# mpitid/babble

Measured on AMD Instinct MI355X. Metric: consensus-ordered events/sec at N participants, higher is better.
Workload: dtype int32; 1 GPU; random-gossip DAG, 256 participants, 10000000 events per GPU, RunConsensus every K=256 events (39063 calls); participants=256, events_per_graph=10000000, k=256, graphs_per_gpu=1, parallelism=replicas1

## Files before the change

### babble_amd/csrc/hge_engine.hip

```cpp
#include <hip/hip_runtime.h>

#include <algorithm>
#include <chrono>
#include <cstdio>
#include <cstdlib>
#include <cstring>
#include <mutex>
#include <optional>
#include <string>
#include <thread>
#include <utility>
#include <vector>

#include "../../include/hge.h"
#include "hge_plan.h"
#include "hge_kernels.hip"
#include "hge_median_rows.hip"
#include "hge_wide32.hip"
#include "hge_coords.hip"
#include "hge_coords_win.hip"
#include "hge_rounds_coop.hip"
#include "hge_rounds_direct.hip"
#include "hge_walk_spec.hip"

// ... 375 lines not shown
    s_lwsum.free_();
    s_lwinit.free_();
    d_ts.free_();
    d_FDTD.free_();
    d_FDTW.free_();
    d_cts.free_();
    s_cts.free_();
    d_S.free_();
    d_ssb.free_();
    d_seeb.free_();
    s_H.free_();
    s_wdbg.free_();
    s_segfws.free_();
    d_coin.free_();
    d_wit.free_();
    d_fame.free_();
    s_dec.free_();
    s_decbit.free_();
    s_segdec.free_();
    s_keys.free_();
    s_keys2.free_();
    d_opcp.free_();
    d_tsch.free_();
    d_LA16.free_();
    d_ssc.free_();
    s_gran.free_();
    s_cH.free_();
    s_cS.free_();
    s_cT.free_();
    s_cM.free_();
    s_cn.free_();
    s_mb.free_();
    s_wpaths.free_();
    s_hist.free_();
    s_hstate.free_();
    s_hssc.free_();
    if (pin) (void)hipHostFree(pin);
    pin = nullptr;
    pin_cap = pin_used = 0;
    if (pin_ord) (void)hipHostFree(pin_ord);
    pin_ord = nullptr;
    pin_ord_dev = nullptr;
    pin_ord_cap = 0;
    cons_pin_n = 0;
    if (st) (void)hipStreamDestroy(st);
    st = nullptr;
  }

  void ensure_events(int64_t m) {
    if (m <= Ecap) return;
    int64_t cap = std::max<int64_t>(m, Ecap + Ecap / 2);
    d_creator.grow_keep(cap, n_dev, st);
    d_index.grow_keep(cap, n_dev, st);
    d_sp.grow_keep(cap, n_dev, st);
    d_op.grow_keep(cap, n_dev, st);
    d_ntx.grow_keep(cap, n_dev, st);
    d_ts.grow_keep(cap, n_dev, st);
    d_S.grow_keep(4 * cap, 4 * n_dev, st);
    d_coin.grow_keep(cap, n_dev, st);
    d_round.grow_keep(cap, n_coords, st);
    d_wit.grow_keep(cap, n_coords, st);
    d_rr.grow_keep(cap, n_coords, st, 0xFF);
    d_cts.grow_keep(cap, n_coords, st, 0);
    d_und.grow_keep(cap, n_und, st);
    Ecap = cap;
  }
// ... 938 lines not shown
      const char* mf = getenv("HGE_TEST_DIR_MEMBER_FLAG");
      int mflag_ep = mf ? atoi(mf) : 0;
      void* dargs[] = {&t, &olen, &len, &rstate, &rlo, &rlo_dev, &Rprev, &gran, &err, &ssc, &mb, &dbg,
                       &nostart, &nohist, &hmax, &nostart, &extra, &stall_ep, &force_exact, &mflag_ep, &paths,
                       &paths_next};
      prof_begin("k_rounds_direct");
      HIPCHK(launch_resident(direct_fn(), dim3(N), dim3(1024), dargs));
      prof_end();
    } else {
      void* args[] = {&t, &FDT, &olen, &len, &rstate, &rlo, &rlo_dev, &Rprev, &gran, &err, &ssc, &dbg};
      prof_begin("k_rounds_coop");
      HIPCHK(launch_resident((const void*)k_rounds_coop, dim3(N), dim3(COOP_BS), args));
      prof_end();
    }
    if (getenv("HGE_TEST_HANDOFF_FAIL")) {
      const int32_t one = 1, down = hge_plan::kRoundsStoodDown;
      h2d(err, &one, 4);
      h2d(rstate + 1, &down, 4);
    }
  }
  uint32_t* walk_mb() {
    s_mb.need((size_t)npow() * npow() + (size_t)npow() * npow() / 2);
    return s_mb.p;
  }
  DBuf<unsigned long long> s_wpaths;
  int walk_seq = 0;
  unsigned long long* walk_paths() {
    if (!s_wpaths.p) {
      s_wpaths.need(4);
      HIPCHK(hipMemset(s_wpaths.p, 0, 4 * sizeof(unsigned long long)));
    }
    walk_seq++;
    return s_wpaths.p + 2 * (walk_seq & 1);
  }
  static int walk_force_exact() {
    const char* e = getenv("HGE_TEST_DIR_EXACT");
    return e && atoi(e) != 0 ? 1 : 0;
  }
  const void* direct_fn() const {
    return N <= 64 ? (const void*)k_rounds_direct<1024, 64>
         : N <= 128 ? (const void*)k_rounds_direct<1024, 128>
                    : (const void*)k_rounds_direct<1024, 256>;
  }

  bool sweep16() const { return N > 32 && !wide32; }
  bool wla16() const { return N > 192 && (N & 3) == 0 && !wide32; }

  void to_wide32() {
    auto test_stop = [&](int stage) {
      if (test_w32_fail == stage) {
        test_w32_fail = 0;
        throw EngineError(HGE_ERR_DEVICE, "test: to_wide32 stopped after stage " + std::to_string(stage));
      }
    };
    ensure_fdtd();
    if (!(w32_done & 4)) {
      grow_chain_table(d_LA, ccap, false);
      w32_done |= 4;
      test_stop(1);
    }
    if (fdt16()) {
      const size_t n = (size_t)N * N * ccap;
      for (int which = 0; which < 2; which++) {
        if (w32_done & (1 << which)) continue;
        DBuf<int32_t>& b = which ? d_FD : d_FDT;
        int32_t* q = nullptr;
// ... 561 lines not shown
    oc.cand = b.cand;
    oc.ncand = ncand;
    oc.R_last = b.R_last;
    oc.recv = s_recv.p;
    oc.rr = s_rr.p;
    oc.cts = s_cts.p;
    oc.cnt = out_counts();
    oc.bpos = s_bpos.p;
    oc.total = out_word(hge_plan::ResultsLayout::kReceived);
    oc.blist = s_bpos.p + ncalls;
    oc.nblist = s_bpos.p + 2 * ncalls;
    oc.f_und = s_fund.p;
    oc.upos = s_upos.p;
    oc.nund = out_word(hge_plan::ResultsLayout::kUndetermined);
    oc.und_out = s_und2.p;
    oc.k1 = (OKey*)s_keys.p;
    oc.k2 = (OKey*)s_keys2.p;
    oc.ev_rr = d_rr.p;
    oc.ev_cts = d_cts.p;
    oc.ntx = out_tx(b);
    oc.ntxb = b.out.ntxb;
    oc.ids = out_ids(b);
    oc.pr = c_pr;
    oc.nrounds = b.do_fame ? b.w.nrounds() : 0;
    oc.clast = s_clast.p;
    oc.dec = s_dec.p;
    oc.nc = c_nc;
    oc.flags = c_flags;
    oc.lcr_old = lcr;
    oc.n_lo = (int)std::min<int64_t>(b.calls[0], n_coords);
    oc.n1 = (int)n_coords;
    oc.lcre_out = out_word(hge_plan::ResultsLayout::kLcrEvents);
    oc.front = front;
    return oc;
  }

  void ensure_wla(Batch& b) {
    if (b.wla_done || N <= 16 || b.R_last <= b.rr_lo) return;
    b.wla_done = true;
    d_WLA.need((size_t)Rcap * N * N);
    if (N > 64 && !wide32) d_WLR.need((size_t)Rcap * N * N);
    const Tables tw = tables();
    KLAUNCH(k_witness_la, dim3(div_up(N, 64), div_up(N, 64), b.R_last - b.rr_lo), dim3(256), 0, st, tw, b.rr_lo);
  }

  void order_stages(Batch& b) {
    const int ncalls = b.ncalls, ncand = b.ncand, nr = b.nr, nrounds = b.w.nrounds();
    s_out.need(b.out.total());
    const bool ocall = nr > 0 && ncalls == 1 && b.calls[0] >= n_coords && b.commit && N <= 16 && !b.spl &&
                       ncand <= SCAN_LDS && (int64_t)nr * group_lanes() <= 65536 && (nrounds == 0 || b.lcr_dev) &&
                       !getenv("HGE_NO_ORDER_CALL");
    if (!ocall) launch_pending_fame(b);
    if (nr == 0) {
      if (!b.hdr_done) out_init(b);
      s_recv.need(ncand);
      HIPCHK(hipMemsetAsync(s_recv.p, 0xFF, 4 * ncand, st));
      return;
    }
    SegInfo& si = b.si;
    si.pr_index = c_pidx;
    if (nrounds > 0) {
      si.pr_off = c_pr + nrounds;
      si.pr_cf = c_pr + 2 * nrounds;
      si.pr_len = c_pr + 3 * nrounds;
      si.clast = s_clast.p;
      si.dec = s_dec.p;
// ... 111 lines not shown
    if (!rlu)
      KLAUNCH(k_recv_flags, dim3(div_up(ncand, 256)), dim3(256), 0, st, s_recv.p, ncand,
              (int32_t*)nullptr, s_fund.p, b.commit ? 1 : 0, b.commit ? o_cc : (int32_t*)nullptr);
    if (!b.commit) {
      KLAUNCH(k_set_rr, dim3(div_up(ncand, 256)), dim3(256), 0, st, t, cand, ncand, s_recv.p,
              s_rr.p, s_cts.p, d_rr.p, d_cts.p, (unsigned long long*)out_word(hge_plan::ResultsLayout::kTx), 0);
      return;
    }
    s_bpos.need(2 * (size_t)ncalls + 2);
    int32_t* blist = s_bpos.p + ncalls;
    int32_t* nblist = s_bpos.p + 2 * ncalls;
    const bool lu = ncand <= 16384;
    s_und2.need(d_und.n);
    if (rlu)
      KLAUNCH(k_recv_list_und, dim3(2), dim3(1024), 0, st, (const int32_t*)s_recv.p, (int)ncand, o_cc, ncalls,
              s_bpos.p, o_cnt, blist, nblist, s_fund.p, s_upos.p, o_und, cand, s_und2.p);
    else if (lu)
      KLAUNCH(k_list_und, dim3(2), dim3(1024), 0, st, (const int32_t*)o_cc, ncalls, s_bpos.p, o_cnt, blist,
              nblist, (const int32_t*)s_fund.p, s_upos.p, (int)ncand, o_und, cand, s_und2.p);
    else
      KLAUNCH(k_bucket_list, dim3(1), dim3(1024), 0, st, (const int32_t*)o_cc, ncalls, s_bpos.p,
              o_cnt, blist, nblist);
    s_keys.need((size_t)ncand * sizeof(OKey));
    s_keys2.need((size_t)ncand * sizeof(OKey));
    OKey* k1 = (OKey*)s_keys.p;
    OKey* k2 = (OKey*)s_keys2.p;
    KLAUNCH(k_bucket_keys, dim3(div_up(ncand, 256)), dim3(256), 0, st, t, cand, ncand, s_recv.p,
            s_rr.p, s_cts.p, s_bpos.p, k1, d_rr.p, d_cts.p, out_tx(b));
    int32_t* ids_dst = out_ids(b);
    if (lazy_order && !b.order_out && !b.spl && pin_ord_dev) {
      ids_dst = pin_ord_dev;
      b.wrote_direct = true;
    }
    if (ncalls <= 8) {
      KLAUNCH(k_bucket_sort_all, dim3(ncalls), dim3(1024), 0, st, (const int32_t*)s_bpos.p,
              (const int32_t*)o_cc, (const int32_t*)blist, (const int32_t*)nblist, k1, k2, ids_dst);
    } else {
      KLAUNCH(k_bucket_sort, dim3(std::min(ncalls, 2048)), dim3(256), 0, st,
              (const int32_t*)s_bpos.p, (const int32_t*)o_cc, (const int32_t*)blist,
              (const int32_t*)nblist, k1, k2, ids_dst, 1);
      if (ncand > 512)
        KLAUNCH(k_bucket_sort_big, dim3(std::min(ncalls, n_cu())), dim3(1024), 0, st,
                (const int32_t*)s_bpos.p, (const int32_t*)o_cc, (const int32_t*)blist,
                (const int32_t*)nblist, (const OKey*)k1, k2, ids_dst);
    }
    if (!lu) {
      scan_large(s_fund.p, s_upos.p, ncand, o_und);
      KLAUNCH(k_scatter_und, dim3(div_up(ncand, 256)), dim3(256), 0, st, cand, ncand, s_fund.p, s_upos.p,
              s_und2.p);
    }
    std::swap(d_und, s_und2);
    b.got_order = true;
  }

  void persist_fame(Batch& b) {
    const int nrounds = b.w.nrounds();
    if (!b.do_fame || nrounds == 0 || b.order_ran != OrderRan::Stages) return;
    const Tables t = tables();
    int32_t* const lcre_out = out_word(hge_plan::ResultsLayout::kLcrEvents);
    if (b.lcr_dev) {
      const int64_t nfrom = std::min<int64_t>(b.calls[0], n_coords);
      const int nb_fp = (int)div_up((int64_t)nrounds * N, 256);
      KLAUNCH(k_fame_persist_lcre, dim3(nb_fp + std::max(1, div_up(n_coords - nfrom, 256))), dim3(256), 0, st, t,
              (const int32_t*)c_pr, (const int32_t*)(c_pr + nrounds), (const int32_t*)(c_pr + 2 * nrounds),
              (const int32_t*)(c_pr + 3 * nrounds), nrounds, (const int32_t*)s_clast.p, (const uint8_t*)s_dec.p,
              nb_fp, (const int64_t*)c_nc, (const int32_t*)c_flags, lcr, (int)nfrom, (int)n_coords, lcre_out);
      return;
    }
    fame_persist(t, nrounds);
    if (b.lcr_new > lcr) {
      b.lcr_up = true;
      const int r = b.lcr_new - 1;
      if (r >= 0) {
        const int64_t nfrom = std::min<int64_t>(b.calls[b.c_set], n_coords);
        KLAUNCH(k_lcre, dim3(std::max(1, div_up(n_coords - nfrom, 256))), dim3(256), 0, st, t,
                (int)nfrom, (int)n_coords, r, lcre_out);
      }
// ... 1311 lines not shown
  h->prof_names.clear();
  h->prof_ms.clear();
  h->prof_cnt.clear();
  return HGE_OK;
}

int hge_kernel_stats(hge_engine* h, int k, char* name, int namecap, double* total_ms,
                     int64_t* launches) {
  const int n = (int)h->prof_names.size();
  if (k < 0 || k >= n) return n;
  if (name && namecap > 0) {
    snprintf(name, namecap, "%s", h->prof_names[k].c_str());
  }
  if (total_ms) *total_ms = h->prof_ms[k];
  if (launches) *launches = h->prof_cnt[k];
  return n;
}

int32_t hge_coordinate_sweeps(hge_engine* h) { return h ? h->n_sweeps : -1; }

int hge_walk_select_paths(hge_engine* h, int64_t* narrow, int64_t* exact) {
  GUARD_BEGIN
  unsigned long long v[2] = {0, 0};
  if (h->s_wpaths.p && h->walk_seq > 0) {
    h->d2h(v, h->s_wpaths.p + 2 * (h->walk_seq & 1), 16);
    h->sync();
  }
  if (narrow) *narrow = (int64_t)v[0];
  if (exact) *exact = (int64_t)v[1];
  return HGE_OK;
  GUARD_END(h)
}

int64_t hge_host_syncs(hge_engine* h) { return h ? h->n_syncs : -1; }

int hge_stage_times(hge_engine* h, float* ms_out, int cap) {
  int n = std::min(cap, 7);
  for (int i = 0; i < n; i++) ms_out[i] = h->stage_ms[i];
  return n;
}

int64_t hge_frontier_fallbacks(hge_engine* h) {
  if (!h) return HGE_ERR_ARG;
  return h->n_frontier_fallbacks;
}

}
```

### babble_amd/csrc/hge_kernels.hip

```cpp
#include <hip/hip_runtime.h>
#include <stdint.h>

#define INF32 0x7FFFFFFF

namespace hge {

struct Tables {
  int N, NW, SM, ccap, Rcap;
  int NW2;
  uint32_t* LA16;
  const int32_t* creator;
  const int32_t* index;
  const int32_t* sp;
  const int32_t* op;
  const int64_t* ts;
  const uint64_t* S;
  const uint8_t* coin;
  const int32_t* ntx;
  int32_t* chain;
  int2* opcp;
  int64_t* tsch;
  int32_t* FDTD;
  uint8_t* FDTW;
  int32_t* WLA;
  uint16_t* WLA16;
  uint16_t* WLR;
  int32_t* LA;
  int32_t* FD;
  uint16_t* FD16;
  int32_t* round;
  uint8_t* wit;
  int32_t* C;
  int32_t* W;
  uint64_t* ssb;
// ... 2423 lines not shown
      sb[i] = k.b;
      ss[i] = (uint32_t)(k.s0 >> 32);
    } else {
      sr[i] = 0xFFFFFFFFu;
      sb[i] = ~0ull;
      ss[i] = 0xFFFFFFFFu;
    }
    ix[i] = (uint16_t)i;
  }
  __syncthreads();
  for (int size = 2; size <= P; size <<= 1) {
    for (int stride = size >> 1; stride > 0; stride >>= 1) {
      for (int i = tid; i < P / 2; i += T) {
        const int lo = 2 * stride * (i / stride) + (i % stride);
        const int hi = lo + stride;
        const bool up = ((lo & size) == 0);
        const int x = ix[lo], y = ix[hi];
        bool yl;
        if (sr[x] != sr[y]) yl = sr[y] < sr[x];
        else if (sb[x] != sb[y]) yl = sb[y] < sb[x];
        else if (ss[x] != ss[y]) yl = ss[y] < ss[x];
        else if (x >= n || y >= n) yl = y < x;
        else yl = okless(K[y], K[x]);
        if (yl == up) {
          ix[lo] = (uint16_t)y;
          ix[hi] = (uint16_t)x;
        }
      }
      bitonic_sync(stride, stride > 1 ? stride >> 1 : size);
    }
  }
}

__device__ void bucket_sort_big_one(int b, int nb, const int32_t* bend, const OKey* keys, OKey* tmp,
                                    int32_t* ids_out, uint64_t* sb, uint32_t* sr, uint32_t* ss, uint16_t* ix) {
  const int tid = threadIdx.x, T = blockDim.x;
  {
    const OKey* K = keys + (bend[b] - nb);
    int32_t* out = ids_out + (bend[b] - nb);
    if (nb <= BIG_SORT) {
      big_bitonic(K, nb, sb, sr, ss, ix);
      for (int i = tid; i < nb; i += T) out[i] = (int32_t)K[ix[i]].id;
      __syncthreads();
      return;
    }
    int32_t* S = (int32_t*)(tmp + (bend[b] - nb));
    const int na = (nb + 1) >> 1, nbb = nb - na;
    big_bitonic(K, na, sb, sr, ss, ix);
    for (int i = tid; i < na; i += T) S[i] = ix[i];
    __syncthreads();
    big_bitonic(K + na, nbb, sb, sr, ss, ix);
    for (int i = tid; i < nbb; i += T) S[na + i] = na + ix[i];
    __syncthreads();
    const int32_t* A = S;
    const int32_t* B = S + na;
    const int k0 = (int)((int64_t)nb * tid / T), k1 = (int)((int64_t)nb * (tid + 1) / T);
    int lo = max(0, k0 - nbb), hi = min(k0, na);
    while (lo < hi) {
      const int i = (lo + hi) >> 1;
      if (okless(K[A[i]], K[B[k0 - i - 1]])) lo = i + 1;
      else hi = i;
    }
    int i = lo, j = k0 - lo;
    for (int k = k0; k < k1; k++) {
      const bool takeA = j >= nbb || (i < na && okless(K[A[i]], K[B[j]]));
      out[k] = (int32_t)K[takeA ? A[i++] : B[j++]].id;
    }
    __syncthreads();
  }
}

__global__ void __launch_bounds__(1024) k_bucket_sort_big(const int32_t* bend, const int32_t* bcnt,
                                                          const int32_t* list, const int32_t* nlist,
                                                          const OKey* keys, OKey* tmp, int32_t* ids_out) {
  __shared__ uint64_t sb[BIG_SORT];
  __shared__ uint32_t sr[BIG_SORT], ss[BIG_SORT];
  __shared__ uint16_t ix[BIG_SORT];
  for (int li = blockIdx.x; li < *nlist; li += gridDim.x) {
    const int b = list[li];
    const int nb = bcnt[b];
    if (nb <= 512 || nb > 2 * BIG_SORT) continue;
    bucket_sort_big_one(b, nb, bend, keys, tmp, ids_out, sb, sr, ss, ix);
  }
}

__global__ void __launch_bounds__(1024) k_bucket_sort_all(const int32_t* bend, const int32_t* bcnt,
                                                          const int32_t* list, const int32_t* nlist,
                                                          OKey* keys, OKey* tmp, int32_t* ids_out) {
  constexpr size_t BIG_LDS = (size_t)BIG_SORT * (8 + 4 + 4 + 2);
  constexpr size_t POOL = BIG_LDS > sizeof(SortChunk<SORT_CH>) ? BIG_LDS : sizeof(SortChunk<SORT_CH>);
  __shared__ __attribute__((aligned(16))) unsigned char pool[POOL];
  uint64_t* sb = (uint64_t*)pool;
  uint32_t* sr = (uint32_t*)(pool + (size_t)BIG_SORT * 8);
  uint32_t* ss = (uint32_t*)(pool + (size_t)BIG_SORT * 12);
  uint16_t* ix = (uint16_t*)(pool + (size_t)BIG_SORT * 16);
  SortChunk<SORT_CH>& sc = *(SortChunk<SORT_CH>*)pool;
  for (int li = blockIdx.x; li < *nlist; li += gridDim.x) {
    const int b = list[li];
    const int nb = bcnt[b];
    if (nb > 512 && nb <= 2 * BIG_SORT) bucket_sort_big_one(b, nb, bend, keys, tmp, ids_out, sb, sr, ss, ix);
    else bucket_sort_one(b, bend, bcnt, keys, tmp, ids_out, false, sc);
    __syncthreads();
  }
}

__global__ void k_scatter_und(const int32_t* cand, int ncand, const int32_t* f_und,
                              const int32_t* pos, int32_t* und) {
  const int q = blockIdx.x * blockDim.x + threadIdx.x;
  if (q >= ncand || !f_und[q]) return;
  und[pos[q]] = cand[q];
}

__global__ void k_set_rr(Tables t, const int32_t* cand, int ncand, const int32_t* recv_call,
                         const int32_t* rr, const int64_t* cts, int32_t* ev_rr, int64_t* ev_cts,
                         unsigned long long* ntx_sum, int commit) {
  const int q = blockIdx.x * blockDim.x + threadIdx.x;
  const bool rec = q < ncand && recv_call[q] >= 0;
  unsigned long long tx = 0;
  if (rec) {
    const int x = cand[q];
    ev_rr[x] = rr[q];
    ev_cts[x] = cts[q];
    tx = (unsigned long long)t.ntx[x];
  }
  if (!commit) return;
  for (int o = 32; o > 0; o >>= 1) tx += __shfl_xor(tx, o);
  if ((threadIdx.x & 63) == 0 && tx) atomicAdd(ntx_sum, tx);
}

__global__ void k_split_filter(const int32_t* cand, int ncand, int32_t* recv_call, int c_lo, int c_hi,
                               int32_t guard, int32_t* flag) {
  const int q = blockIdx.x * blockDim.x + threadIdx.x;
  bool bad = false;
// ... 95 lines not shown
  if ((int)blockIdx.x < nb_fp) fame_persist_body(t, pr_round, pr_off, pr_cf, pr_len, nrounds, clast, dec, blockIdx.x);
  else lcre_dev_body(t, nc, flags, lcr_old, n_lo, n1, out, blockIdx.x - nb_fp);
}

struct OrderCall {
  SegInfo si;
  int rr_lo, nr;
  const int32_t* segoff;
  int32_t *segcnt, *seg_call, *seg_round;
  uint8_t* seg_dec;
  uint64_t* seg_fws;
  int32_t* theta;
  const int32_t* cand;
  int ncand, R_last;
  int32_t *recv, *rr;
  int64_t* cts;
  int32_t *cnt, *bpos, *total, *blist, *nblist;
  int32_t *f_und, *upos, *nund, *und_out;
  OKey *k1, *k2;
  int32_t* ev_rr;
  int64_t* ev_cts;
  unsigned long long* ntx;
  int ntxb;
  int32_t* ids;
  const int32_t* pr;
  int nrounds;
  const int32_t* clast;
  const uint8_t* dec;
  const int64_t* nc;
  const int32_t* flags;
  int lcr_old, n_lo, n1;
  int32_t* lcre_out;
  int front;
};
constexpr size_t OC_BIG_LDS = (size_t)BIG_SORT * (8 + 4 + 4 + 2);
constexpr size_t OC_POOL = OC_BIG_LDS > sizeof(SortChunk<SORT_CH>) ? OC_BIG_LDS : sizeof(SortChunk<SORT_CH>);
static_assert(OC_POOL >= sizeof(int) * (SCAN_LDS + SCAN_LDS / 16), "the scan borrows the sort pool");
template <int G>
__device__ __forceinline__ void order_call_body(const Tables& t, const OrderCall& o, unsigned char* pool) {
  __shared__ int s_cnt;
  __shared__ unsigned long long s_tx[16];
  const int tid = threadIdx.x, T = blockDim.x;
  if (o.front) {
    for (int64_t b = 0; b < (int64_t)o.nr * G; b += T)
      segments_group<G, 1>(t, b + tid, o.rr_lo, o.nr, 1, nullptr, o.si, o.segoff, o.segcnt, o.seg_call,
                           o.seg_round, o.seg_dec, o.seg_fws, o.theta);
    __syncthreads();
    for (int q = tid; q < o.ncand; q += T)
      round_received_item<1>(t, q, o.cand, o.ncand, nullptr, 1, 0, o.rr_lo, o.R_last, o.segoff, o.segcnt,
                             o.seg_call, o.seg_dec, o.seg_fws, o.theta, o.recv, o.rr, o.cts, nullptr);
  }
  if (tid == 0) s_cnt = 0;
  __syncthreads();
  int c = 0;
  for (int q = tid; q < o.ncand; q += T) c += o.recv[q] >= 0 ? 1 : 0;
  for (int s2 = 32; s2 > 0; s2 >>= 1) c += __shfl_xor(c, s2);
  if ((tid & 63) == 0 && c) atomicAdd(&s_cnt, c);
  for (int q = tid; q < o.ncand; q += T) o.f_und[q] = o.recv[q] == -1 ? 1 : 0;
  __syncthreads();
  if (tid == 0) o.cnt[0] = s_cnt;
  __syncthreads();
  bucket_list_body(o.cnt, 1, o.bpos, o.total, o.blist, o.nblist);
  __syncthreads();
  scan_small_core(o.f_und, o.upos, o.ncand, o.nund, o.cand, o.und_out, (int*)pool);
  __syncthreads();
  unsigned long long tx = 0;
  for (int b = 0; b < o.ncand; b += T)
    tx += bucket_key_item(t, b + tid, o.cand, o.ncand, o.recv, o.rr, o.cts, o.bpos, o.k1, o.ev_rr, o.ev_cts);
  if ((tid & 63) == 0) s_tx[tid >> 6] = tx;
  __syncthreads();
  if (tid == 0) {
    unsigned long long bt = 0;
    for (int w = 0; w < T / 64; w++) bt += s_tx[w];
    o.ntx[0] = bt;
  }
  for (int i = 1 + tid; i < o.ntxb; i += T) o.ntx[i] = 0;
  __syncthreads();
  {
    uint64_t* sb = (uint64_t*)pool;
    uint32_t* sr = (uint32_t*)(pool + (size_t)BIG_SORT * 8);
    uint32_t* ss = (uint32_t*)(pool + (size_t)BIG_SORT * 12);
    uint16_t* ix = (uint16_t*)(pool + (size_t)BIG_SORT * 16);
    SortChunk<SORT_CH>& sc = *(SortChunk<SORT_CH>*)pool;
    const int nl = *o.nblist;
    for (int li = 0; li < nl; li++) {
      const int b = o.blist[li];
      const int nb = o.cnt[b];
      if (nb > 512 && nb <= 2 * BIG_SORT) bucket_sort_big_one(b, nb, o.bpos, o.k1, o.k2, o.ids, sb, sr, ss, ix);
      else bucket_sort_one(b, o.bpos, o.cnt, o.k1, o.k2, o.ids, false, sc);
      __syncthreads();
    }
  }
  if (o.nrounds > 0) {
    const int np = o.nrounds;
    for (int b = 0; (int64_t)b * T < (int64_t)np * t.N; b++)
      fame_persist_body(t, o.pr, o.pr + np, o.pr + 2 * np, o.pr + 3 * np, np, o.clast, o.dec, b);
    for (int b = 0; b == 0 || b * T < o.n1 - o.n_lo; b++)
      lcre_dev_body(t, o.nc, o.flags, o.lcr_old, o.n_lo, o.n1, o.lcre_out, b);
  }
}
template <int G>
__global__ void __launch_bounds__(1024) k_order_call(Tables t, OrderCall o) {
  __shared__ __attribute__((aligned(16))) unsigned char pool[OC_POOL];
  order_call_body<G>(t, o, pool);
}
template <int G>
__global__ void __launch_bounds__(1024) k_consensus_call(Tables t, FameCall f, OrderCall o) {
  __shared__ __attribute__((aligned(16))) unsigned char pool[OC_POOL];
  fame_call_body<G, 1, true>(t, f);
  __syncthreads();
  order_call_body<G>(t, o, pool);
}

struct DynCall {
  int lcr, ncand, Rcap;
  int64_t n_c;
  const int32_t* rstate;
  const int32_t* minw;
  int64_t* c_nc;
  int32_t *c_Rc, *c_Lc, *c_flags, *c_pr, *c_pidx, *c_sgo;
  uint8_t *dec, *decbit;
// ... 143 lines not shown
```

### babble_amd/engine.py

```python
import ctypes
import os

import numpy as np

_ROOT = os.path.dirname(os.path.dirname(os.path.abspath(__file__)))
LIB_PATH = os.environ.get("HGE_LIB", os.path.join(_ROOT, "build", "libhge.so"))

HGE_NONE = -1
HGE_UNKNOWN = -2

ERRORS = {
    -1: "Could not find fake creator id",
    -2: "Self-parent not known",
    -3: "Self-parent has different creator",
    -4: "Other-parent not known",
    -5: "Self-parent not last known event by creator",
    -6: "Event index does not match the creator's chain position",
    -7: "Chain capacity exceeded",
    -11: "too late",
    -12: "not found",
}
HGE_ERR_CAPACITY = -7
HGE_ERR_TOO_LATE = -11
HGE_ERR_NOT_FOUND = -12
# ... 6 lines not shown

class HgeEvent(ctypes.Structure):
    _fields_ = [
        ("creator", ctypes.c_int32),
        ("index", ctypes.c_int32),
        ("self_parent", ctypes.c_int32),
        ("other_parent", ctypes.c_int32),
        ("timestamp_ns", ctypes.c_int64),
        ("s", ctypes.c_uint8 * 32),
        ("hash", ctypes.c_uint8 * 32),
        ("n_tx", ctypes.c_int32),
        ("reserved", ctypes.c_int32),
    ]


EVENT_DTYPE = np.dtype([
    ("creator", "<i4"), ("index", "<i4"), ("self_parent", "<i4"), ("other_parent", "<i4"),
    ("timestamp_ns", "<i8"), ("s", "u1", (32,)), ("hash", "u1", (32,)), ("n_tx", "<i4"),
    ("reserved", "<i4"),
])
assert EVENT_DTYPE.itemsize == ctypes.sizeof(HgeEvent)

EXPORTS = [
    "hge_create", "hge_destroy", "hge_last_error", "hge_reset", "hge_insert_events",
    "hge_divide_rounds", "hge_decide_fame", "hge_decide_round_received", "hge_find_order",
    "hge_run_consensus", "hge_replay", "hge_replay_prepare", "hge_replay_run",
    "hge_replay_fetch", "hge_replay_order", "hge_event_count", "hge_participants", "hge_rounds",
    "hge_last_consensus_round", "hge_last_committed_round_events",
    "hge_consensus_transactions", "hge_consensus_count", "hge_consensus_events",
    "hge_undetermined", "hge_known", "hge_round_of", "hge_is_witness", "hge_round_witness",
    "hge_fame", "hge_round_events", "hge_round_received", "hge_consensus_timestamp",
    "hge_consensus_timestamp_sources",
    "hge_ancestor", "hge_self_ancestor", "hge_see", "hge_strongly_see",
    "hge_oldest_self_ancestor_to_see", "hge_coordinates", "hge_coordinate_sweeps", "hge_walk_select_paths", "hge_host_syncs", "hge_frontier_fallbacks",
    "hge_stage_times",
    "hge_set_profiling", "hge_reset_kernel_stats", "hge_kernel_stats",
    "hge_consensus_log", "hge_event_rounds", "hge_event_received", "hge_set_cache_size",
    "hge_cache_size", "hge_participant_events", "hge_participant_event", "hge_last_from",
    "hge_diff", "hge_wire_info", "hge_read_wire_parents", "hge_parent_round", "hge_round_inc",
    "hge_round_diff", "hge_set_round", "hge_round_event_ids", "hge_split_begin", "hge_frontier_guess",
    "hge_frontier_walk", "hge_split_finish", "hge_frontier_rows", "hge_split_plan", "hge_split_exchange", "hge_split_run", "hge_split_emulate",
    "hge_verify_events", "hge_sha256_batch", "hge_ingest", "hge_fame_table",
    "hge_sha256_batch_device", "hge_ecdsa_p256_verify_digests_device", "hge_verify_events_device",
    "hge_ingest_device", "hge_device",
    "hge_store_create", "hge_store_destroy", "hge_store_set_event", "hge_store_has_event",
    "hge_store_participant_events", "hge_store_participant_event", "hge_store_last_from",
    "hge_store_known", "hge_store_add_consensus_event", "hge_store_consensus_events",
    "hge_store_consensus_count", "hge_store_set_round", "hge_store_get_round", "hge_store_rounds",
    "hge_store_round_witnesses", "hge_store_round_events",
    "hge_batch_create", "hge_batch_destroy", "hge_batch_last_error", "hge_batch_add", "hge_batch_stage",
    "hge_batch_run", "hge_batch_graphs", "hge_batch_info", "hge_batch_results", "hge_batch_kernel_ms",
    "hge_batch_fallbacks", "hge_batch_set_delivery", "hge_batch_delivery", "hge_batch_commits_view",
    "hge_gob_encode_wire_events", "hge_gob_decode_wire_events", "hge_gob_encode_event_body",
]

_lib = None


class BatchCommits(ctypes.Structure):
    _fields_ = [("ids", ctypes.POINTER(ctypes.c_int32)), ("rr", ctypes.POINTER(ctypes.c_int32)),
                ("cts", ctypes.POINTER(ctypes.c_int64)), ("counts", ctypes.POINTER(ctypes.c_int64)),
                ("ordered", ctypes.c_int64), ("calls", ctypes.c_int64)]


class _HostView:

    def __init__(self, owner, pointer, n, typestr):
# ... 36 lines not shown
        getattr(L, f).argtypes = [vp, P(i32), i64, P(i64)]
    L.hge_replay.argtypes = [vp, ctypes.c_void_p, i64, P(i64), i64, P(i32), P(i32), i64, P(i64),
                             P(i64)]
    L.hge_replay_prepare.argtypes = [vp, ctypes.c_void_p, i64, P(i64), i64, P(i32)]
    L.hge_replay_run.argtypes = [vp, P(i64)]
    L.hge_replay_fetch.argtypes = [vp, P(i32), i64, P(i64)]
    L.hge_replay_order.argtypes = [vp, P(P(i32)), P(i64)]
    for f in ("hge_event_count", "hge_consensus_transactions", "hge_consensus_count"):
        getattr(L, f).argtypes = [vp]
        getattr(L, f).restype = i64
    for f in ("hge_participants", "hge_rounds", "hge_last_consensus_round",
              "hge_last_committed_round_events"):
        getattr(L, f).argtypes = [vp]
        getattr(L, f).restype = i32
    for f in ("hge_consensus_events", "hge_undetermined"):
        getattr(L, f).argtypes = [vp, P(i32), i64]
        getattr(L, f).restype = i64
    L.hge_known.argtypes = [vp, P(i32)]
    for f in ("hge_round_of", "hge_is_witness", "hge_round_events", "hge_round_received"):
        getattr(L, f).argtypes = [vp, i32]
        getattr(L, f).restype = i32
    L.hge_consensus_timestamp.argtypes = [vp, i32]
    L.hge_consensus_timestamp.restype = i64
    for f in ("hge_round_witness", "hge_fame", "hge_ancestor", "hge_self_ancestor", "hge_see",
              "hge_strongly_see", "hge_oldest_self_ancestor_to_see"):
        getattr(L, f).argtypes = [vp, i32, i32]
        getattr(L, f).restype = i32
    L.hge_coordinates.argtypes = [vp, i32, P(i32), P(i32)]
    L.hge_stage_times.argtypes = [vp, P(ctypes.c_float), ctypes.c_int]
    L.hge_coordinate_sweeps.restype = ctypes.c_int32
    L.hge_coordinate_sweeps.argtypes = [vp]
    if hasattr(L, "hge_walk_select_paths"):
        L.hge_walk_select_paths.argtypes = [vp, P(i64), P(i64)]
    if hasattr(L, "hge_gob_encode_wire_events"):
        L.hge_gob_encode_wire_events.argtypes = [vp, i64, P(ctypes.c_uint8), P(i64), i32, P(ctypes.c_uint8), i64,
                                                 P(i64)]
        L.hge_gob_decode_wire_events.argtypes = [P(ctypes.c_uint8), i64, vp, i64, P(ctypes.c_uint8), i64, P(i64),
                                                 i64, P(i64), P(i64), P(i64)]
        L.hge_gob_encode_event_body.argtypes = [vp, P(ctypes.c_uint8), P(i64), P(ctypes.c_uint8), P(i64), i32,
                                                P(ctypes.c_uint8), i64, P(i64)]
    if hasattr(L, "hge_host_syncs"):
        L.hge_host_syncs.restype = i64
        L.hge_host_syncs.argtypes = [vp]
    L.hge_frontier_fallbacks.restype = i64
    L.hge_frontier_fallbacks.argtypes = [vp]
    L.hge_consensus_log.argtypes = [vp, i64, P(i32), i64]
    L.hge_consensus_log.restype = i64
    L.hge_event_rounds.argtypes = [vp, P(i32), P(ctypes.c_uint8), i64]
    L.hge_event_received.argtypes = [vp, P(i32), P(i64), i64]
    L.hge_consensus_timestamp_sources.argtypes = [vp, P(i32), i64, P(i32)]
    L.hge_fame_table.argtypes = [vp, i32, P(ctypes.c_int8)]
    L.hge_fame_table.restype = i32
    L.hge_set_cache_size.argtypes = [vp, i64]
    L.hge_cache_size.argtypes = [vp]
    L.hge_cache_size.restype = i64
    L.hge_participant_events.argtypes = [vp, i32, i64, P(i32), i64, P(i64)]
    L.hge_participant_event.argtypes = [vp, i32, i64]
    L.hge_participant_event.restype = i32
    L.hge_last_from.argtypes = [vp, i32]
    L.hge_last_from.restype = i32
    L.hge_diff.argtypes = [vp, P(i32), P(i32), i64, P(i64)]
    L.hge_wire_info.argtypes = [vp, i32, P(i32)]
    L.hge_read_wire_parents.argtypes = [vp, i32, i32, i32, i32, P(i32), P(i32)]
    L.hge_parent_round.argtypes = [vp, i32]
    L.hge_parent_round.restype = i32
    L.hge_round_inc.argtypes = [vp, i32]
# ... 475 lines not shown
    def split_finish(self, rows, ssc, natural):
        rows = np.ascontiguousarray(rows, np.int32)
        ssc = np.ascontiguousarray(ssc, np.uint64)
        n = ctypes.c_int64()
        self._check(self.L.hge_split_finish(self.h, _p32(rows),
                                            ssc.ctypes.data_as(ctypes.POINTER(ctypes.c_uint64)),
                                            len(rows), 1 if natural else 0, ctypes.byref(n)))
        self._nordered = n.value
        return n.value

    def set_profiling(self, on=True):
        self.L.hge_set_profiling(self.h, 1 if on else 0)
        self.L.hge_reset_kernel_stats(self.h)

    def kernel_stats(self):
        out = {}
        n = self.L.hge_kernel_stats(self.h, -1, None, 0, None, None)
        buf = ctypes.create_string_buffer(128)
        for k in range(n):
            ms = ctypes.c_double()
            cnt = ctypes.c_int64()
            self.L.hge_kernel_stats(self.h, k, buf, 128, ctypes.byref(ms), ctypes.byref(cnt))
            out[buf.value.decode()] = (ms.value, cnt.value)
        return out

    def coordinate_sweeps(self):
        return self.L.hge_coordinate_sweeps(self.h)

    def walk_select_paths(self):
        nar, ex = ctypes.c_int64(), ctypes.c_int64()
        self._check(self.L.hge_walk_select_paths(self.h, ctypes.byref(nar), ctypes.byref(ex)))
        return nar.value, ex.value

    def host_syncs(self):
        return int(self.L.hge_host_syncs(self.h))

    def frontier_fallbacks(self):
        return int(self.L.hge_frontier_fallbacks(self.h))

    def stage_times(self):
        out = (ctypes.c_float * 7)()
        n = self.L.hge_stage_times(self.h, out, 7)
        return list(out)[:n]

    def event_count(self):
        return self.L.hge_event_count(self.h)

    def rounds(self):
        return self.L.hge_rounds(self.h)

    def last_consensus_round(self):
        r = self.L.hge_last_consensus_round(self.h)
        return None if r < 0 else r

    def last_committed_round_events(self):
        return self.L.hge_last_committed_round_events(self.h)

    def consensus_transactions(self):
        return self.L.hge_consensus_transactions(self.h)

    def consensus_events(self):
        m = self.L.hge_consensus_events(self.h, None, 0)
        out = np.zeros(max(1, m), np.int32)
        self.L.hge_consensus_events(self.h, _p32(out), m)
        return out[:m]

# ... 271 lines not shown
```

### include/hge.h

```cpp
#ifndef HGE_H
#define HGE_H

#include <stdint.h>

#ifdef __cplusplus
extern "C" {
#endif

typedef struct hge_engine hge_engine;

enum hge_status {
  HGE_OK = 0,
  HGE_ERR_CREATOR = -1,
  HGE_ERR_SELF_PARENT_UNKNOWN = -2,
  HGE_ERR_SELF_PARENT_CREATOR = -3,
  HGE_ERR_OTHER_PARENT_UNKNOWN = -4,
  HGE_ERR_SELF_PARENT_NOT_LAST = -5,
  HGE_ERR_INDEX = -6,
  HGE_ERR_CAPACITY = -7,
  HGE_ERR_ARG = -8,
  HGE_ERR_DEVICE = -9,
  HGE_ERR_INTERNAL = -10,
  HGE_ERR_TOO_LATE = -11,
  HGE_ERR_NOT_FOUND = -12,
// ... 175 lines not shown
typedef struct {
  int64_t unix_sec;
  int32_t nsec;
  int16_t offset_min;
  int16_t set;
} hge_gob_time;
typedef struct {
  int64_t self_parent_index, other_parent_creator_id, other_parent_index, creator_id, index;
  hge_gob_time timestamp;
  uint8_t r[32], s[32];
  int32_t r_set, s_set;
  int64_t tx_first;
  int32_t tx_count, pad;
} hge_wire_event;
typedef struct {
  int32_t tx_count, n_parents;
  const uint8_t* creator;
  int64_t creator_len;
  hge_gob_time timestamp;
  int64_t index;
} hge_gob_body;
int hge_gob_encode_wire_events(const hge_wire_event* ev, int64_t n, const uint8_t* tx, const int64_t* tx_off,
                               int32_t first_type_id, uint8_t* out, int64_t cap, int64_t* n_out);
int hge_gob_decode_wire_events(const uint8_t* buf, int64_t len, hge_wire_event* ev, int64_t cap_ev, uint8_t* tx,
                               int64_t cap_bytes, int64_t* tx_off, int64_t cap_tx, int64_t* n_ev, int64_t* n_tx,
                               int64_t* n_bytes);
int hge_gob_encode_event_body(const hge_gob_body* body, const uint8_t* tx, const int64_t* tx_off,
                              const uint8_t* parents, const int64_t* parent_off, int32_t first_type_id,
                              uint8_t* out, int64_t cap, int64_t* n_out);

int hge_stage_times(hge_engine* h, float* ms_out, int cap);
int32_t hge_coordinate_sweeps(hge_engine* h);
int hge_walk_select_paths(hge_engine* h, int64_t* narrow, int64_t* exact);
int64_t hge_host_syncs(hge_engine* h);
int64_t hge_frontier_fallbacks(hge_engine* h);
int hge_set_profiling(hge_engine* h, int on);
int hge_reset_kernel_stats(hge_engine* h);
int hge_kernel_stats(hge_engine* h, int k, char* name, int namecap, double* total_ms,
                     int64_t* launches);

#ifdef __cplusplus
}
#endif
#endif
```

Baseline: 225.7 million events/s.

## Sort big buckets with packed 64-bit keys and register bitonic network

Adds a packed-key bitonic sort for large buckets. The round, b and upper s0 fields are range-compressed into one 64-bit word plus a 16-bit index, and the sort runs mostly in registers with DPP and permlane exchanges, using LDS only for transposes. Ties fall back to full OKey comparison, and buckets whose ranges don't fit fall back to the old index bitonic. k_bucket_sort_big now claims buckets dynamically through an atomic counter, and path counters are exposed via hge_sort_paths. The cost is extra reduction passes, tie-break global reads, and atomics per bucket.

```diff
diff --git a/babble_amd/csrc/hge_engine.hip b/babble_amd/csrc/hge_engine.hip
--- a/babble_amd/csrc/hge_engine.hip
+++ b/babble_amd/csrc/hge_engine.hip
@@ -431,6 +431,7 @@
     s_cn.free_();
     s_mb.free_();
     s_wpaths.free_();
+    s_spaths.free_();
     s_hist.free_();
     s_hstate.free_();
     s_hssc.free_();
@@ -1435,6 +1436,20 @@
     }
     walk_seq++;
     return s_wpaths.p + 2 * (walk_seq & 1);
+  }
+  DBuf<unsigned long long> s_spaths;
+  int sort_seq = 0;
+  bool sort_counted = false;
+  SortCtl sort_ctl() {
+    if (!s_spaths.p) {
+      s_spaths.need(8);
+      HIPCHK(hipMemset(s_spaths.p, 0, 8 * sizeof(unsigned long long)));
+    }
+    sort_seq++;
+    sort_counted = true;
+    const char* e = getenv("HGE_TEST_SORT_INDEX");
+    return SortCtl{s_spaths.p + 4 * (sort_seq & 1), s_spaths.p + 4 * ((sort_seq + 1) & 1),
+                   e && atoi(e) != 0 ? 1 : 0};
   }
   static int walk_force_exact() {
     const char* e = getenv("HGE_TEST_DIR_EXACT");
@@ -2062,6 +2077,7 @@
     oc.n1 = (int)n_coords;
     oc.lcre_out = out_word(hge_plan::ResultsLayout::kLcrEvents);
     oc.front = front;
+    oc.sort = sort_ctl();
     return oc;
   }
 
@@ -2239,9 +2255,10 @@
       ids_dst = pin_ord_dev;
       b.wrote_direct = true;
     }
+    sort_counted = false;
     if (ncalls <= 8) {
       KLAUNCH(k_bucket_sort_all, dim3(ncalls), dim3(1024), 0, st, (const int32_t*)s_bpos.p,
-              (const int32_t*)o_cc, (const int32_t*)blist, (const int32_t*)nblist, k1, k2, ids_dst);
+              (const int32_t*)o_cc, (const int32_t*)blist, (const int32_t*)nblist, k1, k2, ids_dst, sort_ctl());
     } else {
       KLAUNCH(k_bucket_sort, dim3(std::min(ncalls, 2048)), dim3(256), 0, st,
               (const int32_t*)s_bpos.p, (const int32_t*)o_cc, (const int32_t*)blist,
@@ -2249,7 +2266,7 @@
       if (ncand > 512)
         KLAUNCH(k_bucket_sort_big, dim3(std::min(ncalls, n_cu())), dim3(1024), 0, st,
                 (const int32_t*)s_bpos.p, (const int32_t*)o_cc, (const int32_t*)blist,
-                (const int32_t*)nblist, (const OKey*)k1, k2, ids_dst);
+                (const int32_t*)nblist, (const OKey*)k1, k2, ids_dst, sort_ctl());
     }
     if (!lu) {
       scan_large(s_fund.p, s_upos.p, ncand, o_und);
@@ -3627,6 +3644,19 @@
   GUARD_END(h)
 }
 
+int hge_sort_paths(hge_engine* h, int64_t* packed, int64_t* index) {
+  GUARD_BEGIN
+  unsigned long long v[2] = {0, 0};
+  if (h->s_spaths.p && h->sort_counted) {
+    h->d2h(v, h->s_spaths.p + 4 * (h->sort_seq & 1), 16);
+    h->sync();
+  }
+  if (packed) *packed = (int64_t)v[0];
+  if (index) *index = (int64_t)v[1];
+  return HGE_OK;
+  GUARD_END(h)
+}
+
 int64_t hge_host_syncs(hge_engine* h) { return h ? h->n_syncs : -1; }
 
 int hge_stage_times(hge_engine* h, float* ms_out, int cap) {
diff --git a/babble_amd/csrc/hge_kernels.hip b/babble_amd/csrc/hge_kernels.hip
--- a/babble_amd/csrc/hge_kernels.hip
+++ b/babble_amd/csrc/hge_kernels.hip
@@ -1,5 +1,7 @@
 #include <hip/hip_runtime.h>
 #include <stdint.h>
+
+#include "hge_sortkey.h"
 
 #define INF32 0x7FFFFFFF
 
@@ -2489,26 +2491,252 @@
   }
 }
 
-__device__ void bucket_sort_big_one(int b, int nb, const int32_t* bend, const OKey* keys, OKey* tmp,
-                                    int32_t* ids_out, uint64_t* sb, uint32_t* sr, uint32_t* ss, uint16_t* ix) {
-  const int tid = threadIdx.x, T = blockDim.x;
+constexpr size_t BIG_LDS = (size_t)BIG_SORT * (8 + 4 + 4 + 2);
+
+__device__ __forceinline__ bool pk_less(uint64_t wa, uint32_t ia, uint64_t wb, uint32_t ib, const OKey* K, int n) {
+  if (wa != wb) return wa < wb;
+  if (ia >= (uint32_t)n || ib >= (uint32_t)n) return ia < ib;
+  const uint64_t* x = (const uint64_t*)&K[ia];
+  const uint64_t* y = (const uint64_t*)&K[ib];
+#pragma unroll 1
+  for (int f = 0; f < 6; f++) {
+    const uint64_t xf = x[f], yf = y[f];
+    if (xf != yf) return xf < yf;
+  }
+  return K[ia].id < K[ib].id;
+}
+static_assert(sizeof(OKey) == 56 && offsetof(OKey, id) == 48, "pk_less walks a .. s3 as six words");
+
+template <int CTRL>
+__device__ __forceinline__ uint32_t pk_dpp(uint32_t v) {
+  return (uint32_t)__builtin_amdgcn_mov_dpp((int)v, CTRL, 0xF, 0xF, true);
+}
+template <int X>
+__device__ __forceinline__ uint32_t pk_xor(uint32_t v, int lane) {
+  if constexpr (X == 1) {
+    return pk_dpp<0xB1>(v);
+  } else if constexpr (X == 2) {
+    return pk_dpp<0x4E>(v);
+  } else if constexpr (X == 4) {
+    return pk_dpp<0x1B>(pk_dpp<0x141>(v));
+  } else if constexpr (X == 8) {
+    return pk_dpp<0x128>(v);
+  } else if constexpr (X == 16) {
+    const auto r = __builtin_amdgcn_permlane16_swap(v, v, false, false);
+    return (lane & 16) ? r[0] : r[1];
+  } else {
+    const auto r = __builtin_amdgcn_permlane32_swap(v, v, false, false);
+    return (lane & 32) ? r[0] : r[1];
+  }
+}
+
+template <int E, int X>
+__device__ __forceinline__ void pk_lane_stage_x(uint64_t (&w)[E], uint32_t (&id)[E], int lane, uint32_t pos, int size,
+                                                const OKey* K, int n) {
+  const bool want_min = ((lane & X) == 0) == ((pos & (uint32_t)size) == 0);
+#pragma unroll
+  for (int e = 0; e < E; e++) {
+    const uint64_t ow = (uint64_t)pk_xor<X>((uint32_t)w[e], lane) | ((uint64_t)pk_xor<X>((uint32_t)(w[e] >> 32), lane) << 32);
+    const uint32_t oi = pk_xor<X>(id[e], lane);
+    const bool take = pk_less(ow, oi, w[e], id[e], K, n) == want_min;
+    w[e] = take ? ow : w[e];
+    id[e] = take ? oi : id[e];
+  }
+}
+template <int E>
+__device__ __forceinline__ void pk_lane_stage(uint64_t (&w)[E], uint32_t (&id)[E], int x, int lane, uint32_t pos,
+                                              int size, const OKey* K, int n) {
+  switch (x) {
+    case 1: pk_lane_stage_x<E, 1>(w, id, lane, pos, size, K, n); break;
+    case 2: pk_lane_stage_x<E, 2>(w, id, lane, pos, size, K, n); break;
+    case 4: pk_lane_stage_x<E, 4>(w, id, lane, pos, size, K, n); break;
+    case 8: pk_lane_stage_x<E, 8>(w, id, lane, pos, size, K, n); break;
+    case 16: pk_lane_stage_x<E, 16>(w, id, lane, pos, size, K, n); break;
+    default: pk_lane_stage_x<E, 32>(w, id, lane, pos, size, K, n); break;
+  }
+}
+
+template <int E>
+__device__ __forceinline__ bool packed_bitonic(const OKey* K, int n, int P, unsigned char* pool, uint16_t* ix) {
+  int tid = threadIdx.x;
+  asm volatile("" : "+v"(tid));
+  const int lane = tid & 63, wv = tid >> 6;
+  const int NT = P / E;
+  const bool act = tid < NT;
+  uint32_t rmin = 0xFFFFFFFFu, rmax = 0;
+  uint64_t bmin = ~0ull, bmax = 0;
+#pragma unroll
+  for (int e = 0; e < E; e++) {
+    const int i = tid * E + e;
+    if (act && i < n) {
+      const uint32_t r = (uint32_t)K[i].a;
+      const uint64_t b = K[i].b;
+      rmin = min(rmin, r);
+      rmax = max(rmax, r);
+      bmin = b < bmin ? b : bmin;
+      bmax = b > bmax ? b : bmax;
+    }
+  }
+  for (int o = 32; o > 0; o >>= 1) {
+    rmin = min(rmin, (uint32_t)__shfl_xor(rmin, o));
+    rmax = max(rmax, (uint32_t)__shfl_xor(rmax, o));
+    const uint64_t a = __shfl_xor(bmin, o), b = __shfl_xor(bmax, o);
+    bmin = a < bmin ? a : bmin;
+    bmax = b > bmax ? b : bmax;
+  }
+  uint64_t* red = (uint64_t*)pool;
+  if (lane == 0) {
+    red[4 * wv] = rmin;
+    red[4 * wv + 1] = rmax;
+    red[4 * wv + 2] = bmin;
+    red[4 * wv + 3] = bmax;
+  }
+  __syncthreads();
+  for (int v = 0; v < (int)(blockDim.x >> 6); v++) {
+    rmin = min(rmin, (uint32_t)red[4 * v]);
+    rmax = max(rmax, (uint32_t)red[4 * v + 1]);
+    bmin = red[4 * v + 2] < bmin ? red[4 * v + 2] : bmin;
+    bmax = red[4 * v + 3] > bmax ? red[4 * v + 3] : bmax;
+  }
+  __syncthreads();
+  const hge_sortkey::SkPlan plan = hge_sortkey::sk_plan(rmin, rmax, bmin, bmax);
+  if (!plan.packable) return false;
+  uint64_t w[E];
+  uint32_t id[E];
+#pragma unroll
+  for (int e = 0; e < E; e++) {
+    const int i = tid * E + e;
+    w[e] = act && i < n ? hge_sortkey::sk_word(plan, (uint32_t)K[i].a, K[i].b, K[i].s0) : hge_sortkey::kSkPad;
+    id[e] = (uint32_t)i;
+  }
+  const int m = (NT >> 6) - 1;
+  const int ptid = ((lane & m) << 6) | (lane & ~m) | (wv & m);
+  const uint32_t posA = (uint32_t)tid * E, posB = (uint32_t)ptid * E;
+  constexpr int LR = 1024;
+  uint64_t* const lw = (uint64_t*)pool;
+  uint64_t* const li = lw + E * LR;
+  auto slot = [](int t) { return (t & ~63) | ((t ^ (t >> 6)) & 63); };
+  auto transpose = [&]() {
+    if (act) {
+      const int s = slot(tid);
+#pragma unroll
+      for (int e = 0; e < E; e++) lw[e * LR + s] = w[e];
+#pragma unroll
+      for (int g = 0; g < E / 4; g++)
+        li[g * LR + s] = (uint64_t)id[4 * g] | ((uint64_t)id[4 * g + 1] << 16) | ((uint64_t)id[4 * g + 2] << 32) |
+                         ((uint64_t)id[4 * g + 3] << 48);
+    }
+    __syncthreads();
+    if (act) {
+      const int s = slot(ptid);
+#pragma unroll
+      for (int e = 0; e < E; e++) w[e] = lw[e * LR + s];
+#pragma unroll
+      for (int g = 0; g < E / 4; g++) {
+        const uint64_t v = li[g * LR + s];
+        id[4 * g] = (uint32_t)v & 0xFFFFu;
+        id[4 * g + 1] = (uint32_t)(v >> 16) & 0xFFFFu;
+        id[4 * g + 2] = (uint32_t)(v >> 32) & 0xFFFFu;
+        id[4 * g + 3] = (uint32_t)(v >> 48);
+      }
+    }
+    __syncthreads();
+  };
+  for (int size = 2; size <= P; size <<= 1) {
+    int j = size >> 1;
+    if (j >= 64 * E) {
+      transpose();
+      if (act)
+        for (; j >= 64 * E; j >>= 1) pk_lane_stage<E>(w, id, j / (64 * E), lane, posB, size, K, n);
+      transpose();
+      j = 32 * E;
+    }
+    if (act) {
+      for (; j >= E; j >>= 1) pk_lane_stage<E>(w, id, j / E, lane, posA, size, K, n);
+#pragma unroll
+      for (int s = E / 2; s >= 1; s >>= 1) {
+        if (s >= size) continue;
+#pragma unroll
+        for (int lo = 0; lo < E; lo++) {
+          if (lo & s) continue;
+          const int hi = lo | s;
+          const bool up = ((posA + lo) & (uint32_t)size) == 0;
+          if (pk_less(w[hi], id[hi], w[lo], id[lo], K, n) == up) {
+            const uint64_t tw = w[lo];
+            w[lo] = w[hi];
+            w[hi] = tw;
+            const uint32_t ti = id[lo];
+            id[lo] = id[hi];
+            id[hi] = ti;
+          }
+        }
+      }
+    }
+  }
+  if (act) {
+#pragma unroll
+    for (int g = 0; g < E / 4; g++)
+      ((uint64_t*)ix)[tid * (E / 4) + g] = (uint64_t)id[4 * g] | ((uint64_t)id[4 * g + 1] << 16) |
+                                           ((uint64_t)id[4 * g + 2] << 32) | ((uint64_t)id[4 * g + 3] << 48);
+  }
+  __syncthreads();
+  return true;
+}
+
+struct SortCtl {
+  unsigned long long* cur;
+  unsigned long long* next;
+  int force_index;
+};
+__device__ __forceinline__ void sort_ctl_begin(const SortCtl& c) {
+  if (blockIdx.x == 0 && threadIdx.x == 0 && c.next) c.next[0] = c.next[1] = c.next[2] = 0;
+}
+
+__device__ __forceinline__ bool big_sort_keys(const OKey* K, int n, unsigned char* pool, bool force_index) {
+  uint16_t* ix = (uint16_t*)(pool + (size_t)BIG_SORT * 16);
+  if (!force_index) {
+    int P = 1024;
+    while (P < n) P <<= 1;
+    if (P <= 4096 ? packed_bitonic<4>(K, n, P, pool, ix) : packed_bitonic<8>(K, n, P, pool, ix)) return true;
+  }
+  big_bitonic(K, n, (uint64_t*)pool, (uint32_t*)(pool + (size_t)BIG_SORT * 8),
+              (uint32_t*)(pool + (size_t)BIG_SORT * 12), ix);
+  return false;
+}
+
+__device__ __forceinline__ void bucket_sort_big_one(int b, int nb, const int32_t* bend, const OKey* keys, OKey* tmp,
+                                    int32_t* ids_out, unsigned char* pool, const SortCtl& ctl) {
+  const int T = blockDim.x;
+  const uint16_t* ix = (const uint16_t*)(pool + (size_t)BIG_SORT * 16);
+  const bool fi = ctl.force_index != 0;
+  auto thread = []() {
+    int t = threadIdx.x;
+    asm volatile("" : "+v"(t));
+    return t;
+  };
   {
-    const OKey* K = keys + (bend[b] - nb);
-    int32_t* out = ids_out + (bend[b] - nb);
-    if (nb <= BIG_SORT) {
-      big_bitonic(K, nb, sb, sr, ss, ix);
-      for (int i = tid; i < nb; i += T) out[i] = (int32_t)K[ix[i]].id;
+    nb = __builtin_amdgcn_readfirstlane(nb);
+    const int start = __builtin_amdgcn_readfirstlane(bend[b] - nb);
+    const OKey* K = keys + start;
+    int32_t* out = ids_out + start;
+    int32_t* S = (int32_t*)(tmp + start);
+    const bool whole = nb <= BIG_SORT;
+    const int na = whole ? nb : (nb + 1) >> 1, nbb = nb - na;
+    bool pk = true;
+    for (int h = 0; h < (whole ? 1 : 2); h++) {
+      const int off = h ? na : 0, len = h ? nbb : na;
+      pk = big_sort_keys(K + off, len, pool, fi) && pk;
+      const int tid = thread();
+      if (whole) {
+        for (int i = tid; i < len; i += T) out[i] = (int32_t)K[ix[i]].id;
+      } else {
+        for (int i = tid; i < len; i += T) S[off + i] = off + ix[i];
+      }
       __syncthreads();
-      return;
-    }
-    int32_t* S = (int32_t*)(tmp + (bend[b] - nb));
-    const int na = (nb + 1) >> 1, nbb = nb - na;
-    big_bitonic(K, na, sb, sr, ss, ix);
-    for (int i = tid; i < na; i += T) S[i] = ix[i];
-    __syncthreads();
-    big_bitonic(K + na, nbb, sb, sr, ss, ix);
-    for (int i = tid; i < nbb; i += T) S[na + i] = na + ix[i];
-    __syncthreads();
+    }
+    const int tid = thread();
+    if (tid == 0 && ctl.cur) atomicAdd(&ctl.cur[pk ? 0 : 1], 1ull);
+    if (whole) return;
     const int32_t* A = S;
     const int32_t* B = S + na;
     const int k0 = (int)((int64_t)nb * tid / T), k1 = (int)((int64_t)nb * (tid + 1) / T);
@@ -2529,33 +2757,35 @@
 
 __global__ void __launch_bounds__(1024) k_bucket_sort_big(const int32_t* bend, const int32_t* bcnt,
                                                           const int32_t* list, const int32_t* nlist,
-                                                          const OKey* keys, OKey* tmp, int32_t* ids_out) {
-  __shared__ uint64_t sb[BIG_SORT];
-  __shared__ uint32_t sr[BIG_SORT], ss[BIG_SORT];
-  __shared__ uint16_t ix[BIG_SORT];
+                                                          const OKey* keys, OKey* tmp, int32_t* ids_out, SortCtl ctl) {
+  __shared__ __attribute__((aligned(16))) unsigned char pool[BIG_LDS];
+  __shared__ int s_li;
+  sort_ctl_begin(ctl);
+  const int nl = *nlist;
+  for (;;) {
+    if (threadIdx.x == 0) s_li = (int)atomicAdd(&ctl.cur[2], 1ull);
+    __syncthreads();
+    const int li = s_li;
+    __syncthreads();
+    if (li >= nl) break;
+    const int b = list[li];
+    const int nb = bcnt[b];
+    if (nb <= 512 || nb > 2 * BIG_SORT) continue;
+    bucket_sort_big_one(b, nb, bend, keys, tmp, ids_out, pool, ctl);
+  }
+}
+
+__global__ void __launch_bounds__(1024) k_bucket_sort_all(const int32_t* bend, const int32_t* bcnt,
+                                                          const int32_t* list, const int32_t* nlist,
+                                                          OKey* keys, OKey* tmp, int32_t* ids_out, SortCtl ctl) {
+  constexpr size_t POOL = BIG_LDS > sizeof(SortChunk<SORT_CH>) ? BIG_LDS : sizeof(SortChunk<SORT_CH>);
+  __shared__ __attribute__((aligned(16))) unsigned char pool[POOL];
+  SortChunk<SORT_CH>& sc = *(SortChunk<SORT_CH>*)pool;
+  sort_ctl_begin(ctl);
   for (int li = blockIdx.x; li < *nlist; li += gridDim.x) {
     const int b = list[li];
     const int nb = bcnt[b];
-    if (nb <= 512 || nb > 2 * BIG_SORT) continue;
-    bucket_sort_big_one(b, nb, bend, keys, tmp, ids_out, sb, sr, ss, ix);
-  }
-}
-
-__global__ void __launch_bounds__(1024) k_bucket_sort_all(const int32_t* bend, const int32_t* bcnt,
-                                                          const int32_t* list, const int32_t* nlist,
-                                                          OKey* keys, OKey* tmp, int32_t* ids_out) {
-  constexpr size_t BIG_LDS = (size_t)BIG_SORT * (8 + 4 + 4 + 2);
-  constexpr size_t POOL = BIG_LDS > sizeof(SortChunk<SORT_CH>) ? BIG_LDS : sizeof(SortChunk<SORT_CH>);
-  __shared__ __attribute__((aligned(16))) unsigned char pool[POOL];
-  uint64_t* sb = (uint64_t*)pool;
-  uint32_t* sr = (uint32_t*)(pool + (size_t)BIG_SORT * 8);
-  uint32_t* ss = (uint32_t*)(pool + (size_t)BIG_SORT * 12);
-  uint16_t* ix = (uint16_t*)(pool + (size_t)BIG_SORT * 16);
-  SortChunk<SORT_CH>& sc = *(SortChunk<SORT_CH>*)pool;
-  for (int li = blockIdx.x; li < *nlist; li += gridDim.x) {
-    const int b = list[li];
-    const int nb = bcnt[b];
-    if (nb > 512 && nb <= 2 * BIG_SORT) bucket_sort_big_one(b, nb, bend, keys, tmp, ids_out, sb, sr, ss, ix);
+    if (nb > 512 && nb <= 2 * BIG_SORT) bucket_sort_big_one(b, nb, bend, keys, tmp, ids_out, pool, ctl);
     else bucket_sort_one(b, bend, bcnt, keys, tmp, ids_out, false, sc);
     __syncthreads();
   }
@@ -2717,8 +2947,9 @@
   int lcr_old, n_lo, n1;
   int32_t* lcre_out;
   int front;
+  SortCtl sort;
 };
-constexpr size_t OC_BIG_LDS = (size_t)BIG_SORT * (8 + 4 + 4 + 2);
+constexpr size_t OC_BIG_LDS = BIG_LDS;
 constexpr size_t OC_POOL = OC_BIG_LDS > sizeof(SortChunk<SORT_CH>) ? OC_BIG_LDS : sizeof(SortChunk<SORT_CH>);
 static_assert(OC_POOL >= sizeof(int) * (SCAN_LDS + SCAN_LDS / 16), "the scan borrows the sort pool");
 template <int G>
@@ -2762,16 +2993,13 @@
   for (int i = 1 + tid; i < o.ntxb; i += T) o.ntx[i] = 0;
   __syncthreads();
   {
-    uint64_t* sb = (uint64_t*)pool;
-    uint32_t* sr = (uint32_t*)(pool + (size_t)BIG_SORT * 8);
-    uint32_t* ss = (uint32_t*)(pool + (size_t)BIG_SORT * 12);
-    uint16_t* ix = (uint16_t*)(pool + (size_t)BIG_SORT * 16);
     SortChunk<SORT_CH>& sc = *(SortChunk<SORT_CH>*)pool;
+    sort_ctl_begin(o.sort);
     const int nl = *o.nblist;
     for (int li = 0; li < nl; li++) {
       const int b = o.blist[li];
       const int nb = o.cnt[b];
-      if (nb > 512 && nb <= 2 * BIG_SORT) bucket_sort_big_one(b, nb, o.bpos, o.k1, o.k2, o.ids, sb, sr, ss, ix);
+      if (nb > 512 && nb <= 2 * BIG_SORT) bucket_sort_big_one(b, nb, o.bpos, o.k1, o.k2, o.ids, pool, o.sort);
       else bucket_sort_one(b, o.bpos, o.cnt, o.k1, o.k2, o.ids, false, sc);
       __syncthreads();
     }
diff --git a/babble_amd/csrc/hge_sortkey.h b/babble_amd/csrc/hge_sortkey.h
--- /dev/null
+++ b/babble_amd/csrc/hge_sortkey.h
@@ -0,0 +1,46 @@
+#pragma once
+
+#include <stdint.h>
+
+#if defined(__HIPCC__) || defined(__CUDACC__)
+#define HGE_SK_HD __host__ __device__ __forceinline__
+#else
+#define HGE_SK_HD inline
+#endif
+
+namespace hge_sortkey {
+
+constexpr uint64_t kSkPad = ~0ull;
+
+HGE_SK_HD int sk_bits(uint64_t x) {
+  int n = 0;
+  while (x) {
+    n++;
+    x >>= 1;
+  }
+  return n;
+}
+
+struct SkPlan {
+  uint32_t rr_min;
+  uint64_t b_min;
+  int wr, wc;
+  bool packable;
+};
+
+HGE_SK_HD SkPlan sk_plan(uint32_t rr_min, uint32_t rr_max, uint64_t b_min, uint64_t b_max) {
+  SkPlan p;
+  p.rr_min = rr_min;
+  p.b_min = b_min;
+  p.wr = sk_bits((uint64_t)(rr_max - rr_min));
+  p.wc = sk_bits(b_max - b_min);
+  p.packable = p.wr + p.wc <= 32;
+  return p;
+}
+
+HGE_SK_HD uint64_t sk_word(const SkPlan& p, uint32_t rr, uint64_t b, uint64_t s0) {
+  const uint64_t lead = ((uint64_t)(rr - p.rr_min) << p.wc) | (b - p.b_min);
+  return (lead << 32) | (s0 >> 32);
+}
+
+}
diff --git a/babble_amd/engine.py b/babble_amd/engine.py
--- a/babble_amd/engine.py
+++ b/babble_amd/engine.py
@@ -62,7 +62,7 @@
     "hge_fame", "hge_round_events", "hge_round_received", "hge_consensus_timestamp",
     "hge_consensus_timestamp_sources",
     "hge_ancestor", "hge_self_ancestor", "hge_see", "hge_strongly_see",
-    "hge_oldest_self_ancestor_to_see", "hge_coordinates", "hge_coordinate_sweeps", "hge_walk_select_paths", "hge_host_syncs", "hge_frontier_fallbacks",
+    "hge_oldest_self_ancestor_to_see", "hge_coordinates", "hge_coordinate_sweeps", "hge_walk_select_paths", "hge_sort_paths", "hge_host_syncs", "hge_frontier_fallbacks",
     "hge_stage_times",
     "hge_set_profiling", "hge_reset_kernel_stats", "hge_kernel_stats",
     "hge_consensus_log", "hge_event_rounds", "hge_event_received", "hge_set_cache_size",
@@ -165,6 +165,8 @@
     L.hge_coordinate_sweeps.argtypes = [vp]
     if hasattr(L, "hge_walk_select_paths"):
         L.hge_walk_select_paths.argtypes = [vp, P(i64), P(i64)]
+    if hasattr(L, "hge_sort_paths"):
+        L.hge_sort_paths.argtypes = [vp, P(i64), P(i64)]
     if hasattr(L, "hge_gob_encode_wire_events"):
         L.hge_gob_encode_wire_events.argtypes = [vp, i64, P(ctypes.c_uint8), P(i64), i32, P(ctypes.c_uint8), i64,
                                                  P(i64)]
@@ -706,6 +708,11 @@
         self._check(self.L.hge_walk_select_paths(self.h, ctypes.byref(nar), ctypes.byref(ex)))
         return nar.value, ex.value
 
+    def sort_paths(self):
+        pk, ix = ctypes.c_int64(), ctypes.c_int64()
+        self._check(self.L.hge_sort_paths(self.h, ctypes.byref(pk), ctypes.byref(ix)))
+        return pk.value, ix.value
+
     def host_syncs(self):
         return int(self.L.hge_host_syncs(self.h))
 
diff --git a/include/hge.h b/include/hge.h
--- a/include/hge.h
+++ b/include/hge.h
@@ -231,6 +231,7 @@
 int hge_stage_times(hge_engine* h, float* ms_out, int cap);
 int32_t hge_coordinate_sweeps(hge_engine* h);
 int hge_walk_select_paths(hge_engine* h, int64_t* narrow, int64_t* exact);
+int hge_sort_paths(hge_engine* h, int64_t* packed, int64_t* index);
 int64_t hge_host_syncs(hge_engine* h);
 int64_t hge_frontier_fallbacks(hge_engine* h);
 int hge_set_profiling(hge_engine* h, int on);
```

Measured after the change: 230.7 million events/s (median of 6 runs). +2.2%, better.
